# puzzlepaint/camera_calibration

Measured on NVIDIA H100. Metric: LM iterations/sec, higher is better.
Workload: dtype f64

## Files before the change

### camera_calibration_b200/csrc/ba_dense.cu

```cuda

#include <algorithm>
#include <cstdio>
#include <cstdlib>

#include "ba_kernels.h"
#include "ba_tile.cuh"

namespace b200ba {

namespace {

constexpr int BM = 128;
constexpr int LDT = BM + 4;
__host__ __device__ constexpr int gemm_threads(int bn) { return 4 * (bn / 32) * 32; }
constexpr size_t gemm_smem(int bn, int bk, int stages) {
  return static_cast<size_t>(stages) * bk * (LDT + bn + 4) * sizeof(double);
}

__device__ __forceinline__ void cp_async16(void* smem, const void* gmem, int src_bytes) {
  const unsigned s = static_cast<unsigned>(__cvta_generic_to_shared(smem));
  asm volatile("cp.async.cg.shared.global [%0], [%1], 16, %2;\n" ::"r"(s), "l"(gmem), "r"(src_bytes));
}
__device__ __forceinline__ void cp_async8(void* smem, const void* gmem, int src_bytes) {
  const unsigned s = static_cast<unsigned>(__cvta_generic_to_shared(smem));
// ... 598 lines not shown
      bs[row] = v;
    else if (live_row)
      b_below[r] = v;
  }
  if (!chain) return;
  cp_async_wait<0>();
  __syncthreads();
  double s0 = 0.0, s1 = 0.0;
  for (int c = half; c <= row; c += 4) {
    s0 = fma(ts2_smem[c * TS2_LD + row], bs[c], s0);
    if (c + 2 <= row) s1 = fma(ts2_smem[(c + 2) * TS2_LD + row], bs[c + 2], s1);
  }
  part[half][row] = s0 + s1;
  __syncthreads();
  if (half == 0 && live_row) y_next[row] = part[0][row] + part[1][row];
}

__global__ void __launch_bounds__(TS2_THREADS, 1)
    trsv_backward2_kernel(const double* __restrict__ Lpack, const int64_t* __restrict__ panel_off,
                          const int* __restrict__ panel_h, int NB, int r0, int live, const double* __restrict__ x_t,
                          double* __restrict__ y , const double* __restrict__ Linv_prev,
                          double* __restrict__ x_prev ) {
  extern __shared__ __align__(16) double ts2_smem[];
  __shared__ double xs[PT], ysm[PT], part[2][PT];
  const int tid = threadIdx.x;
  const bool chain = blockIdx.x == 0;
  if (chain) stage_tile_async(ts2_smem, Linv_prev);
  if (tid < PT) xs[tid] = (tid < live) ? x_t[tid] : 0.0;
  __syncthreads();
  const int warp = tid >> 5, lane = tid & 31;
  const int cbase = r0 - PT * (static_cast<int>(blockIdx.x) + 1);
#pragma unroll
  for (int batch = 0; batch < 2; ++batch) {
    double l[8][4];
#pragma unroll
    for (int q = 0; q < 8; ++q) {
      const int c = cbase + warp * 16 + batch * 8 + q;
      const int k = c / NB;
      const double* col = Lpack + panel_off[k] + static_cast<int64_t>(c - k * NB) * panel_h[k] + (r0 - k * NB);
#pragma unroll
      for (int u = 0; u < 4; ++u) l[q][u] = (lane + 32 * u < live) ? col[lane + 32 * u] : 0.0;
    }
#pragma unroll
    for (int q = 0; q < 8; ++q) {
      double acc = 0.0;
#pragma unroll
      for (int u = 0; u < 4; ++u) acc = fma(l[q][u], xs[lane + 32 * u], acc);
#pragma unroll
      for (int o = 16; o > 0; o >>= 1) acc += __shfl_xor_sync(0xffffffffu, acc, o);
      if (lane == 0) {
        const int c = cbase + warp * 16 + batch * 8 + q;
        const double v = y[c] - acc;
        if (chain)
          ysm[c - cbase] = v;
        else
          y[c] = v;
      }
    }
  }
  if (!chain) return;
  cp_async_wait<0>();
  __syncthreads();
  const int j = tid & (PT - 1), half = tid >> 7;
  double s0 = 0.0, s1 = 0.0;
  const double* colj = ts2_smem + j * TS2_LD;
  for (int i = j + half; i < PT; i += 4) {
    s0 = fma(colj[i], ysm[i], s0);
    if (i + 2 < PT) s1 = fma(colj[i + 2], ysm[i + 2], s1);
  }
  part[half][j] = s0 + s1;
  __syncthreads();
  if (half == 0) x_prev[j] = part[0][j] + part[1][j];
}

static int panel_version() {
  static int v = -1;
  if (v < 0) v = getenv("B200BA_PANEL") ? atoi(getenv("B200BA_PANEL")) : 2;
  return v;
}
static bool aux_enabled() {
  static const bool v = !(getenv("B200BA_AUX") && atoi(getenv("B200BA_AUX")) == 0);
  return v;
}
static int trsv_version() {
  static int v = -1;
  if (v < 0) v = getenv("B200BA_TRSV") ? atoi(getenv("B200BA_TRSV")) : 2;
  return v;
}

void dense_variants(int* gemm, int* panel, int* trsv, int* aux) {
  *gemm = gemm_variant();
  *panel = panel_version();
  *trsv = trsv_version();
  *aux = aux_enabled() ? 1 : 0;
}

int dense_plan(DenseCtx* d, int n, int nb, int rank, int ranks) {
  d->n = n;
  d->rank = rank;
  d->ranks = ranks;
  d->NB = nb;
  d->nblk = (n + nb - 1) / nb;
  d->ntiles = (n + PT - 1) / PT;
  d->map.nb = nb;
  d->map.ranks = ranks;
  d->map.blocks_per_rank = (d->nblk + ranks - 1) / ranks;
  d->map.ld = (n + 1) / 2 * 2;
  d->chunk = static_cast<int64_t>(d->map.blocks_per_rank) * nb * d->map.ld;
  d->panel_off.assign(d->nblk + 1, 0);
  d->panel_h.assign(std::max(1, d->nblk), 0);
  for (int k = 0; k < d->nblk; ++k) {
    const int hk = n - k * nb;
    d->panel_h[k] = (hk + 1) / 2 * 2;
    d->panel_off[k + 1] = d->panel_off[k] + static_cast<int64_t>(d->panel_h[k]) * nb + static_cast<int64_t>(nb / PT) * PT * PT;
  }
  return 0;
}

int dense_factor(DenseCtx* d) {
  const int n = d->n, NB = d->NB, R = d->ranks, me = d->rank;
  if (n == 0) return 0;
  const int sub_n = NB / PT;
  cudaStream_t sm = d->s_main, sp = d->s_panel;
  auto owner = [&](int k) { return k % R; };
  const bool use_aux = aux_enabled() && R == 1 && d->s_aux != nullptr;
  cudaEventRecord(d->ev_misc, sm);
  cudaStreamWaitEvent(sp, d->ev_misc, 0);

  auto update = [&](int k, int j_first, int j_last, cudaStream_t st, bool owned_only) -> int {
    if (j_first >= d->nblk || j_first > j_last) return 0;
    const int k0 = k * NB, kw = std::min(NB, n - k0);
    const int j0 = j_first * NB;
    const int jn = std::min(n, (std::min(j_last, d->nblk - 1) + 1) * NB) - j0;
    if (jn <= 0) return 0;
    GemmArgs g{};
    g.M = n - j0;
    g.N = jn;
    g.K = kw;
    g.A = d->Lpack + d->panel_off[k] + (j0 - k0);
    g.lda = d->panel_h[k];
    g.B = g.A;
    g.ldb = g.lda;
    g.alpha = -1.0;
    g.beta = 1.0;
    g.a_aligned = g.b_aligned = gemm_operand_aligned(g.A, g.lda);
    if (owned_only) {
      g.C = d->S;
      g.map = d->map;
      g.owned_only = true;
      g.rank = me;
      g.col_base = j0;
    } else {
      g.C = d->S + d->map.col_offset(j0) + j0;
      g.ldc = d->map.ld;
    }
    return launch_dgemm_nt(g, true, false, st, false, true);
  };

  for (int k = 0; k < d->nblk; ++k) {
    const int k0 = k * NB, kw = std::min(NB, n - k0), hk = d->panel_h[k], hlive = n - k0;
    double* P = d->Lpack + d->panel_off[k];
    if (owner(k) == me && panel_version() == 2) {
      const double* Sk = d->S + d->map.col_offset(k0) + k0;
      double* Sk_w = d->S + d->map.col_offset(k0) + k0;
      const int64_t ld = d->map.ld;
      for (int sub = 0; sub < sub_n; ++sub) {
        const int c0 = sub * PT;
        if (c0 >= kw) break;
        const int live = std::min(PT, kw - c0);
        double* tile_out = P + static_cast<int64_t>(c0) * hk + c0;
        double* Li = P + static_cast<int64_t>(hk) * NB + static_cast<int64_t>(sub) * PT * PT;
        if (launch_potrf_trinv_tile(Sk + static_cast<int64_t>(c0) * ld + c0, ld, live, tile_out, hk, Li, d->info, sp)) return 1;
        const int below = hlive - c0 - PT;
        if (below > 0) {
          GemmArgs g{};
          g.M = below;
          g.N = PT;
          g.K = PT;
          g.A = Sk + static_cast<int64_t>(c0) * ld + c0 + PT;
          g.lda = ld;
          g.B = Li;
          g.ldb = PT;
          g.C = tile_out + PT;
          g.ldc = hk;
          g.alpha = 1.0;
          g.beta = 0.0;
          g.a_aligned = gemm_operand_aligned(g.A, g.lda);
          g.b_aligned = gemm_operand_aligned(g.B, g.ldb);
          if (launch_dgemm_nt(g, false, false, sp, false, true)) return 1;
          const int rest = kw - c0 - PT;
          if (rest > 0) {
            GemmArgs u{};
            u.M = below;
            u.N = rest;
            u.K = PT;
            u.A = tile_out + PT;
            u.lda = hk;
            u.B = u.A;
            u.ldb = hk;
            u.C = Sk_w + static_cast<int64_t>(c0 + PT) * ld + (c0 + PT);
            u.ldc = ld;
            u.alpha = -1.0;
            u.beta = 1.0;
            u.a_aligned = u.b_aligned = gemm_operand_aligned(u.A, u.lda);
            if (launch_dgemm_nt(u, true, false, sp, false, true)) return 1;
          }
        }
      }
    } else if (owner(k) == me) {
      cudaMemcpy2DAsync(P, static_cast<size_t>(hk) * sizeof(double), d->S + d->map.col_offset(k0) + k0,
                        static_cast<size_t>(d->map.ld) * sizeof(double), static_cast<size_t>(hlive) * sizeof(double), kw,
                        cudaMemcpyDeviceToDevice, sp);
      for (int sub = 0; sub < sub_n; ++sub) {
        const int c0 = sub * PT;
        if (c0 >= kw) break;
        const int live = std::min(PT, kw - c0);
        double* tile = P + static_cast<int64_t>(c0) * hk + c0;
        double* Li = P + static_cast<int64_t>(hk) * NB + static_cast<int64_t>(sub) * PT * PT;
        if (launch_potrf_tile(tile, hk, live, Li, d->info, sp)) return 1;
        const int below = hlive - c0 - PT;
        if (below > 0) {
          GemmArgs g{};
          g.M = below;
          g.N = PT;
          g.K = PT;
          g.A = tile + PT;
          g.lda = hk;
          g.B = Li;
          g.ldb = PT;
          g.C = tile + PT;
          g.ldc = hk;
          g.alpha = 1.0;
          g.beta = 0.0;
          g.in_place = true;
          g.a_aligned = gemm_operand_aligned(g.A, g.lda);
          g.b_aligned = gemm_operand_aligned(g.B, g.ldb);
          if (launch_dgemm_nt(g, false, false, sp)) return 1;
          const int rest = kw - c0 - PT;
          if (rest > 0) {
            GemmArgs u{};
            u.M = below;
            u.N = rest;
            u.K = PT;
            u.A = tile + PT;
            u.lda = hk;
            u.B = u.A;
            u.ldb = hk;
            u.C = P + static_cast<int64_t>(c0 + PT) * hk + (c0 + PT);
            u.ldc = hk;
            u.alpha = -1.0;
            u.beta = 1.0;
            u.a_aligned = u.b_aligned = gemm_operand_aligned(u.A, u.lda);
            if (launch_dgemm_nt(u, true, false, sp)) return 1;
          }
        }
      }
    }
    if (R > 1) {
      if (d->bcast(P, static_cast<size_t>(hk) * NB + static_cast<size_t>(sub_n) * PT * PT, owner(k), sp, d->user)) return 1;
    }
    cudaEventRecord(d->ev_ready[k & 1], sp);
    cudaStreamWaitEvent(sm, d->ev_ready[k & 1], 0);
    if (k + 3 < d->nblk && update(k, k + 3, d->nblk - 1, sm, R > 1)) return 1;
    cudaEventRecord(d->ev_main[k & 1], sm);
    if (use_aux) {
      if (k >= 1) cudaStreamWaitEvent(sp, d->ev_half2[(k - 1) & 1], 0);
      if (k + 1 < d->nblk && update(k, k + 1, k + 1, sp, false)) return 1;
      if (k + 2 < d->nblk) {
        cudaStreamWaitEvent(d->s_aux, d->ev_ready[k & 1], 0);
        if (k > 0) cudaStreamWaitEvent(d->s_aux, d->ev_main[(k - 1) & 1], 0);
        if (update(k, k + 2, k + 2, d->s_aux, false)) return 1;
      }
      cudaEventRecord(d->ev_half2[k & 1], d->s_aux);
      continue;
    }
    if (k + 1 < d->nblk && owner(k + 1) == me && update(k, k + 1, k + 1, sp, false)) return 1;
    if (k + 2 < d->nblk && owner(k + 2) == me) {
      if (k > 0) cudaStreamWaitEvent(sp, d->ev_main[(k - 1) & 1], 0);
      if (update(k, k + 2, k + 2, sp, false)) return 1;
    }
  }
  if (use_aux && d->nblk >= 1) cudaStreamWaitEvent(sp, d->ev_half2[(d->nblk - 1) & 1], 0);
  cudaEventRecord(d->ev_misc, sp);
  cudaStreamWaitEvent(sm, d->ev_misc, 0);
  return cudaGetLastError() == cudaSuccess ? 0 : 1;
}

int dense_solve(DenseCtx* d, double* b) {
  const int n = d->n, NB = d->NB;
  if (n == 0) return 0;
  cudaStream_t sm = d->s_main;
  const int sub_n = NB / PT;
  auto linv_of = [&](int t) {
    const int k = (t * PT) / NB, sub = (t * PT - k * NB) / PT;
    return d->Lpack + d->panel_off[k] + static_cast<int64_t>(d->panel_h[k]) * NB + static_cast<int64_t>(sub) * PT * PT;
  };
  if (trsv_version() == 2) {
    static bool configured_dev[64] = {};
    int dev = 0;
    cudaGetDevice(&dev);
    if (!configured_dev[dev & 63]) {
      cudaFuncSetAttribute(trsv_forward2_kernel, cudaFuncAttributeMaxDynamicSharedMemorySize, static_cast<int>(kTs2Smem));
      cudaFuncSetAttribute(trsv_backward2_kernel, cudaFuncAttributeMaxDynamicSharedMemorySize, static_cast<int>(kTs2Smem));
      configured_dev[dev & 63] = true;
    }
    const int T = d->ntiles;
    trsv_store_tile_kernel<<<1, PT, 0, sm>>>(linv_of(0), b, std::min(PT, n), d->tmp, false);
    for (int t = 0; t + 1 < T; ++t) {
      const int c0 = t * PT, k = c0 / NB, off = c0 - k * NB;
      const int rows_below = n - c0 - PT;
      const double* Lp = d->Lpack + d->panel_off[k] + static_cast<int64_t>(off) * d->panel_h[k] + off + PT;
      trsv_forward2_kernel<<<(rows_below + PT - 1) / PT, TS2_THREADS, kTs2Smem, sm>>>(Lp, d->panel_h[k], rows_below, d->tmp + c0,
                                                                                      b + c0 + PT, linv_of(t + 1), d->tmp + c0 + PT);
    }
    {
      const int r0 = (T - 1) * PT;
      trsv_store_tile_kernel<<<1, PT, 0, sm>>>(linv_of(T - 1), d->tmp + r0, std::min(PT, n - r0), b + r0, true);
    }
    for (int t = T - 1; t >= 1; --t) {
      const int r0 = t * PT, live = std::min(PT, n - r0);
      trsv_backward2_kernel<<<r0 / PT, TS2_THREADS, kTs2Smem, sm>>>(d->Lpack, d->d_panel_off, d->d_panel_h, NB, r0, live, b + r0,
                                                                    d->tmp, linv_of(t - 1), b + r0 - PT);
    }
    return cudaGetLastError() == cudaSuccess ? 0 : 1;
  }
  for (int t = 0; t < d->ntiles; ++t) {
    const int c0 = t * PT, live = std::min(PT, n - c0), k = c0 / NB;
    const int rows_below = n - c0 - PT;
    const double* Li = linv_of(t);
    if (rows_below > 0) {
      const int grid = (rows_below + TS_ROWS - 1) / TS_ROWS;
      trsv_forward_step_kernel<<<grid, TS_THREADS, 0, sm>>>(d->Lpack + d->panel_off[k], d->panel_h[k], c0 - k * NB, live,
                                                              rows_below, Li, b + c0, d->tmp + c0);
    } else {
      trsv_store_tile_kernel<<<1, PT, 0, sm>>>(Li, b + c0, live, d->tmp + c0, false);
    }
  }
  for (int t = d->ntiles - 1; t >= 0; --t) {
    const int r0 = t * PT, live = std::min(PT, n - r0);
    const double* Li = linv_of(t);
    if (r0 > 0) {
      const int grid = (r0 + TS_THREADS / 32 - 1) / (TS_THREADS / 32);
      trsv_backward_step_kernel<<<grid, TS_THREADS, 0, sm>>>(d->Lpack, d->d_panel_off, d->d_panel_h, NB, r0, live, r0, Li,
                                                               d->tmp + r0, d->tmp, b + r0);
    } else {
      trsv_store_tile_kernel<<<1, PT, 0, sm>>>(Li, d->tmp + r0, live, b + r0, true);
    }
  }
  return cudaGetLastError() == cudaSuccess ? 0 : 1;
}
// ... 58 lines not shown
```

### camera_calibration_b200/csrc/ba_host.cu

```cuda

#include <cublas_v2.h>
#include <cusolverDn.h>
#include <dlfcn.h>

#include <algorithm>
#include <cmath>
#include <cstdarg>
#include <cstdio>
#include <cstring>
#include <limits>
#include <string>
#include <vector>

#include "ba_kernels.h"

using namespace b200ba;

namespace {

std::string g_create_error;

struct NcclUniqueId {
  char internal[128];
};
// ... 59 lines not shown

  std::vector<b200ba_camera> cams_host;
  ProblemDev pb{};
  int n_cameras = 0, n_imagesets = 0, n_points = 0;
  int64_t n_obs = 0;
  int uniform_model = -1;
  int64_t n_control_total = 0, n_param_total = 0, intr_total = 0, tan_total = 0;
  uint32_t *d_obs_imageset = nullptr, *d_obs_camera = nullptr, *d_obs_point = nullptr;
  float2* d_obs_xy = nullptr;

  StateDev st[2]{};
  int cur = 0;
  double2* d_last_projection = nullptr;
  bool have_state = false;
  StateDev snap{};
  double2* d_snap_lp = nullptr;
  bool have_snapshot = false;

  Layout L{};
  bool have_layout = false;
  ObsOut out{};
  ObsOut out_trial{};
  SystemDev sys{};
  double *d_W = nullptr, *d_S = nullptr, *d_Linv = nullptr, *d_v = nullptr, *d_y = nullptr, *d_x = nullptr;
  double trace_H = 0;
  int64_t reduce_count = 0;
  double* d_potrf_work = nullptr;
  int potrf_lwork = 0;
  int chol_mode = -1;
  int chol_nb = 512;
  int *d_info = nullptr, *d_fail = nullptr;
  std::vector<uint32_t> perm;
  uint32_t* d_perm = nullptr;
  double2* d_lp_stage = nullptr;
  uint32_t* d_straggler_list = nullptr;
  int* d_straggler_count = nullptr;
  double *d_partial = nullptr, *d_scal = nullptr;
  double* d_rot = nullptr;
  double* h_scal = nullptr;
  int* h_flags = nullptr;

  std::vector<uint32_t> h_obs_imageset, h_obs_camera, h_obs_point;
  std::vector<float> h_obs_xy;
  int group_blocks_n = 0;
  int n_groups = 0;
  std::vector<int> group_start;
  std::vector<int> group_count;
  int* d_group_of_block = nullptr;
  int* d_group_blocks = nullptr;
  uint8_t* d_flags = nullptr;
  int* d_cols = nullptr;
  int* d_count = nullptr;
  int* h_count = nullptr;
  double* d_Wc = nullptr;
  double* d_P = nullptr;
  size_t wc_stride = 0, p_stride = 0;
  cudaEvent_t ev_syrk[2] = {nullptr, nullptr}, ev_scatter[2] = {nullptr, nullptr}, ev_s_ready = nullptr;
  double* d_u = nullptr;
  bool use_grouped = false;
  double* capture_S = nullptr;
  double* capture_rhs = nullptr;
  std::vector<int32_t> lm_events;
  std::vector<double> grp_sums;
  int force_grouped = -1;
  bool compact_j = true;

  ReportDev rep{};
  double2* d_rep_stage = nullptr;
  bool have_report = false;
  std::vector<int64_t> img_cam_groups;
  int* d_img_group_off = nullptr;
  uint32_t* d_img_group_obs = nullptr;
  bool have_images = false;

  void* comm = nullptr;
  int rank = 0, n_ranks = 1;

  bool own_dense = true;
  DenseCtx dn;
  int dense_planned_ranks = 0, dense_planned_n = -1;
  int dense_nb = 0;
  cudaStream_t panel_stream = nullptr;
  cudaStream_t aux_stream = nullptr;
  int* d_ident_cols = nullptr;
  double* d_gemv_partial = nullptr;

  b200ba_timings timings{};
  struct Pending {
    int phase;
    cudaEvent_t a, b;
    bool own_a = true;
  };
  std::vector<Pending> pending;
  std::vector<cudaEvent_t> event_pool;
};

namespace {

#define CUDA_TRY(h, expr)                                                                      \
  do {                                                                                         \
    cudaError_t _e = (expr);                                                                   \
    if (_e != cudaSuccess) {                                                                   \
      (h)->error = std::string(#expr) + ": " + cudaGetErrorString(_e);                         \
      return 1;                                                                                \
    }                                                                                          \
  } while (0)
#define CUBLAS_TRY(h, expr)                                                                    \
  do {                                                                                         \
    cublasStatus_t _s = (expr);                                                                \
    if (_s != CUBLAS_STATUS_SUCCESS) {                                                         \
      (h)->error = std::string(#expr) + ": cuBLAS status " + std::to_string(static_cast<int>(_s)); \
      return 1;                                                                                \
    }                                                                                          \
  } while (0)
#define CUSOLVER_TRY(h, expr)                                                                  \
  do {                                                                                         \
    cusolverStatus_t _s = (expr);                                                              \
    if (_s != CUSOLVER_STATUS_SUCCESS) {                                                       \
      (h)->error = std::string(#expr) + ": cuSOLVER status " + std::to_string(static_cast<int>(_s)); \
      return 1;                                                                                \
    }                                                                                          \
  } while (0)

template <class T>
int dev_alloc(b200ba_handle* h, T** p, size_t count) {
  if (*p) {
    cudaFree(*p);
    *p = nullptr;
  }
  if (count == 0) count = 1;
  CUDA_TRY(h, cudaMalloc(reinterpret_cast<void**>(p), count * sizeof(T)));
  return 0;
}

int64_t intrinsics_size(const b200ba_camera& c) {
  const int64_t G = static_cast<int64_t>(c.grid_width) * c.grid_height;
  switch (c.model_type) {
    case B200BA_MODEL_CENTRAL_GENERIC: return 3 * G;
    case B200BA_MODEL_NONCENTRAL_GENERIC: return 6 * G;
    default: return 12;
  }
}
int update_parameter_count(const b200ba_camera& c) {
  const int G = c.grid_width * c.grid_height;
  switch (c.model_type) {
    case B200BA_MODEL_CENTRAL_GENERIC: return 2 * G;
    case B200BA_MODEL_NONCENTRAL_GENERIC: return 5 * G;
    default: return 12;
  }
}
int jacobian_size(const b200ba_camera& c) {
  switch (c.model_type) {
    case B200BA_MODEL_CENTRAL_GENERIC: return 32;
    case B200BA_MODEL_NONCENTRAL_GENERIC: return 80;
    default: return 12;
  }
}

void fill_camdev(const b200ba_camera& c, CamDev* d) {
  d->model_type = c.model_type;
  d->width = c.width;
  d->height = c.height;
  d->min_x = c.calibration_min_x;
  d->min_y = c.calibration_min_y;
  d->max_x = c.calibration_max_x;
  d->max_y = c.calibration_max_y;
// ... 71 lines not shown
  cudaFree(d);
  if (rc != 0 || ce != cudaSuccess) {
    h->error = "all-reduce of the group centroids failed";
    return 1;
  }
  return 0;
}

int build_groups(b200ba_handle* h, bool allocate) {
  const Layout& L = h->L;
  const int nb = L.nblocks;
  int gb = (L.bs == 3) ? 96 : 48;
  if (const char* e = getenv("B200BA_GROUP_BLOCKS")) gb = std::max(1, atoi(e));
  h->group_blocks_n = gb;
  std::vector<int> order(nb);
  for (int i = 0; i < nb; ++i) order[i] = i;
  if (L.eliminate_points && nb > 0) {
    const double* sx = h->grp_sums.data();
    const double* sy = sx + nb;
    const double* cnt = sy + nb;
    const double qx = std::max(1.0, h->cams_host[0].width / 64.0), qy = std::max(1.0, h->cams_host[0].height / 64.0);
    std::vector<uint32_t> zkey(nb, 0);
    for (int p = 0; p < nb; ++p) {
      if (cnt[p] <= 0) continue;
      uint32_t ux = static_cast<uint32_t>(std::min(1023.0, std::max(0.0, sx[p] / cnt[p] / qx)));
      uint32_t uy = static_cast<uint32_t>(std::min(1023.0, std::max(0.0, sy[p] / cnt[p] / qy)));
      uint32_t z = 0;
      for (int b = 0; b < 10; ++b) z |= ((ux >> b) & 1u) << (2 * b) | ((uy >> b) & 1u) << (2 * b + 1);
      zkey[p] = z;
    }
    std::stable_sort(order.begin(), order.end(), [&](int a, int b) { return zkey[a] < zkey[b]; });
  }
  h->n_groups = (nb + gb - 1) / gb;
  h->group_start.assign(h->n_groups + 1, 0);
  std::vector<int> gob(std::max(1, nb), 0);
  for (int g = 0; g < h->n_groups; ++g) {
    h->group_start[g] = g * gb;
    for (int i = g * gb; i < std::min(nb, (g + 1) * gb); ++i) gob[order[i]] = g;
  }
  h->group_start[h->n_groups] = nb;
  h->group_count.assign(std::max(1, h->n_groups), 0);
  if (allocate) {
    if (dev_alloc(h, &h->d_group_of_block, std::max(1, nb))) return 1;
    if (dev_alloc(h, &h->d_group_blocks, std::max(1, nb))) return 1;
    if (dev_alloc(h, &h->d_flags, static_cast<size_t>(std::max(1, h->n_groups)) * std::max(1, L.nd))) return 1;
    if (dev_alloc(h, &h->d_cols, static_cast<size_t>(std::max(1, h->n_groups)) * std::max(1, L.nd))) return 1;
    if (dev_alloc(h, &h->d_count, std::max(1, h->n_groups))) return 1;
    if (h->h_count) cudaFreeHost(h->h_count);
    CUDA_TRY(h, cudaMallocHost(reinterpret_cast<void**>(&h->h_count), std::max(1, h->n_groups) * sizeof(int)));
    h->wc_stride = static_cast<size_t>(gb) * L.bs * (std::max(1, L.nd) + 1);
    h->p_stride = static_cast<size_t>(std::max(1, L.nd)) * std::max(1, L.nd);
    if (dev_alloc(h, &h->d_Wc, 2 * h->wc_stride)) return 1;
    if (!h->own_dense && dev_alloc(h, &h->d_P, 2 * h->p_stride)) return 1;
    for (int i = 0; i < 2; ++i) {
      if (!h->ev_syrk[i]) CUDA_TRY(h, cudaEventCreateWithFlags(&h->ev_syrk[i], cudaEventDisableTiming));
      if (!h->ev_scatter[i]) CUDA_TRY(h, cudaEventCreateWithFlags(&h->ev_scatter[i], cudaEventDisableTiming));
    }
    if (!h->ev_s_ready) CUDA_TRY(h, cudaEventCreateWithFlags(&h->ev_s_ready, cudaEventDisableTiming));
    if (dev_alloc(h, &h->d_u, std::max(1, L.nbd))) return 1;
  }
  CUDA_TRY(h, cudaMemcpy(h->d_group_of_block, gob.data(), std::max(1, nb) * sizeof(int), cudaMemcpyHostToDevice));
  if (nb > 0) CUDA_TRY(h, cudaMemcpy(h->d_group_blocks, order.data(), nb * sizeof(int), cudaMemcpyHostToDevice));
  return 0;
}

int nccl_bcast_cb(double* buf, size_t count, int root, cudaStream_t s, void* user) {
  b200ba_handle* h = static_cast<b200ba_handle*>(user);
  const int rc = g_nccl.Broadcast(buf, buf, count, kNcclDouble, root, h->comm, s);
  if (rc != 0) {
    h->error = std::string("ncclBroadcast: ") + (g_nccl.GetErrorString ? g_nccl.GetErrorString(rc) : "error");
    return 1;
  }
  return 0;
}

cudaError_t dense_create(DenseCtx* d, bool own_streams) {
  cudaError_t e = cudaSuccess;
  if (own_streams) {
    int lo = 0, hi = 0;
    cudaDeviceGetStreamPriorityRange(&lo, &hi);
    e = cudaStreamCreateWithFlags(&d->s_main, cudaStreamNonBlocking);
    if (e == cudaSuccess) e = cudaStreamCreateWithPriority(&d->s_panel, cudaStreamNonBlocking, hi);
    if (e == cudaSuccess) e = cudaStreamCreateWithPriority(&d->s_aux, cudaStreamNonBlocking, hi);
  }
  for (cudaEvent_t* ev : {&d->ev_ready[0], &d->ev_ready[1], &d->ev_main[0], &d->ev_main[1], &d->ev_half2[0],
                          &d->ev_half2[1], &d->ev_misc})
    if (e == cudaSuccess && !*ev) e = cudaEventCreateWithFlags(ev, cudaEventDisableTiming);
  return e;
}
void dense_release(DenseCtx* d, bool own_streams) {
  for (cudaEvent_t ev : {d->ev_ready[0], d->ev_ready[1], d->ev_main[0], d->ev_main[1], d->ev_half2[0], d->ev_half2[1],
                         d->ev_misc})
    if (ev) cudaEventDestroy(ev);
  if (own_streams)
    for (cudaStream_t s : {d->s_main, d->s_panel, d->s_aux})
      if (s) cudaStreamDestroy(s);
}

int plan_dense(b200ba_handle* h) {
  if (!h->own_dense || !h->have_layout) return 0;
  const int nd = h->L.nd;
  if (h->dense_planned_n == nd && h->dense_planned_ranks == h->n_ranks) return 0;
  DenseCtx& d = h->dn;
  const int nb = h->dense_nb > 0 ? h->dense_nb : (h->n_ranks == 1 ? 512 : 256);
  dense_plan(&d, nd, nb, h->rank, h->n_ranks);
  if (dev_alloc(h, &h->d_S, static_cast<size_t>(std::max<int64_t>(1, d.chunk * h->n_ranks)))) return 1;
  d.S = h->d_S;
  if (dev_alloc(h, &d.Lpack, static_cast<size_t>(std::max<int64_t>(1, d.panel_off[d.nblk])))) return 1;
  if (dev_alloc(h, &d.tmp, std::max(1, nd))) return 1;
  if (dev_alloc(h, &d.d_panel_off, d.panel_off.size())) return 1;
  if (dev_alloc(h, &d.d_panel_h, d.panel_h.size())) return 1;
  CUDA_TRY(h, cudaMemcpy(d.d_panel_off, d.panel_off.data(), d.panel_off.size() * sizeof(int64_t), cudaMemcpyHostToDevice));
  CUDA_TRY(h, cudaMemcpy(d.d_panel_h, d.panel_h.data(), d.panel_h.size() * sizeof(int), cudaMemcpyHostToDevice));
  {
    std::vector<int> ident(std::max(1, nd));
    for (int i = 0; i < nd; ++i) ident[i] = i;
    if (dev_alloc(h, &h->d_ident_cols, ident.size())) return 1;
    CUDA_TRY(h, cudaMemcpy(h->d_ident_cols, ident.data(), ident.size() * sizeof(int), cudaMemcpyHostToDevice));
  }
  if (dev_alloc(h, &h->d_gemv_partial, static_cast<size_t>(gemv_t_partial_size(h->L.nbd, std::max(1, nd))))) return 1;
  CUDA_TRY(h, cudaMemset(h->d_S, 0, static_cast<size_t>(std::max<int64_t>(1, d.chunk * h->n_ranks)) * sizeof(double)));
  d.info = h->d_info;
  d.s_main = h->stream;
  d.s_panel = h->panel_stream;
  d.s_aux = h->aux_stream;
  CUDA_TRY(h, dense_create(&d, false));
  d.bcast = nccl_bcast_cb;
  d.user = h;
  h->dense_planned_n = nd;
  h->dense_planned_ranks = h->n_ranks;
  return 0;
}

int make_layout(b200ba_handle* h, const b200ba_options* opt) {
  if (opt->regularization_weight != 0) {
    static bool warned = false;
    if (!warned) fprintf(stderr, "[b200ba] regularization_weight is ignored (the term is disabled in the reference, joint_optimization.cc:299-305)\n");
    warned = true;
  }
  Layout L{};
  memset(&L, 0, sizeof(L));
  L.n_points = h->n_points;
  L.n_imagesets = h->n_imagesets;
  L.n_cameras = h->n_cameras;
  L.rig_in_state = h->n_cameras > 1;
  L.localize_only = opt->localize_only ? 1 : 0;
  L.eliminate_points = opt->eliminate_points ? 1 : 0;
  int n_intr = 0, kmax = 0;
  for (int c = 0; c < h->n_cameras; ++c) {
    n_intr += update_parameter_count(h->cams_host[c]);
    kmax = std::max(kmax, jacobian_size(h->cams_host[c]));
  }
  if (L.localize_only) {
    n_intr = 0;
    kmax = 0;
  }
  const int rig_dof = L.rig_in_state ? 6 * h->n_cameras : 0;
  if (L.eliminate_points) {
    L.bs = 3;
    L.nblocks = h->n_points;
    L.g_point = 0;
    L.g_pose = 3 * h->n_points;
    L.g_rig = L.g_pose + 6 * h->n_imagesets;
    L.g_intr = L.g_rig + rig_dof;
  } else {
    L.bs = 6;
    L.nblocks = h->n_imagesets;
    L.g_pose = 0;
    L.g_rig = 6 * h->n_imagesets;
    L.g_point = L.g_rig + rig_dof;
    L.g_intr = L.g_point + 3 * h->n_points;
  }
  L.dsz = L.bs * (L.bs + 1) / 2;
  L.nbd = L.bs * L.nblocks;
  L.dof = 3 * h->n_points + 6 * h->n_imagesets + rig_dof + n_intr;
  L.nd = L.dof - L.nbd;
  L.Kmax = kmax;
  L.jc_point = 0;
  L.jc_pose = 3;
  L.jc_rig = 9;
  L.jc_intr = 9 + (L.rig_in_state ? 6 : 0);
  L.n_jcols = L.jc_intr + kmax;
  const bool same = h->have_layout && memcmp(&L, &h->L, sizeof(Layout)) == 0;
  if (same) return plan_dense(h);
  h->L = L;
  h->have_layout = true;
  h->dense_planned_n = -1;

  const int64_t n = h->n_obs;
  if (dev_alloc(h, &h->out.residual, 2 * n)) return 1;
  if (dev_alloc(h, &h->out.cost, n)) return 1;
  h->out.compact = (h->uniform_model == B200BA_MODEL_CENTRAL_GENERIC && h->compact_j) ? 1 : 0;
  if (h->out.compact) {
    if (h->out.jac) cudaFree(h->out.jac);
    h->out.jac = nullptr;
    if (dev_alloc(h, &h->out.cjac, 14 * static_cast<size_t>(n))) return 1;
  } else {
    if (dev_alloc(h, &h->out.jac, 2 * static_cast<size_t>(L.n_jcols) * n)) return 1;
  }
  if (dev_alloc(h, &h->out.cell, n)) return 1;
  if (dev_alloc(h, &h->out.has_jac, n)) return 1;
  if (dev_alloc(h, &h->out.evals, n)) return 1;
  h->out_trial.evals = nullptr;
  if (dev_alloc(h, &h->out_trial.residual, 2 * n)) return 1;
  if (dev_alloc(h, &h->out_trial.cost, n)) return 1;
  h->out_trial.jac = nullptr;
  h->out_trial.cjac = nullptr;
  h->out_trial.compact = 0;
// ... 915 lines not shown
  }
  cublasSetStream(h->cublas, h->stream);
  if (cusolverDnCreate(&h->cusolver) != CUSOLVER_STATUS_SUCCESS) {
    h->error = "cusolverDnCreate failed";
    return fail(1);
  }
  cusolverDnSetStream(h->cusolver, h->stream);

  h->n_cameras = p->n_cameras;
  h->n_imagesets = p->n_imagesets;
  h->n_points = p->n_points;
  h->n_obs = p->n_obs;
  h->cams_host.assign(p->cameras, p->cameras + p->n_cameras);
  h->uniform_model = h->cams_host[0].model_type;
  int upd = 0;
  for (int c = 0; c < p->n_cameras; ++c) {
    CamDev& d = h->pb.cams[c];
    fill_camdev(h->cams_host[c], &d);
    d.intr_off = h->intr_total;
    d.tan_off = h->tan_total;
    d.upd_off = upd;
    upd += d.upd_count;
    h->intr_total += intrinsics_size(h->cams_host[c]);
    const int64_t G = static_cast<int64_t>(d.gw) * d.gh;
    h->tan_total += 6 * G;
    h->n_control_total += G;
    if (d.gw == 0) h->n_param_total += 12;
    if (h->cams_host[c].model_type != h->uniform_model) h->uniform_model = -1;
  }
  const int64_t n = p->n_obs;
  TRYC(dev_alloc(h, &h->d_obs_imageset, n));
  TRYC(dev_alloc(h, &h->d_obs_camera, n));
  TRYC(dev_alloc(h, &h->d_obs_point, n));
  TRYC(dev_alloc(h, &h->d_obs_xy, n));
  if (n > 0) {
    std::vector<uint32_t> key(n);
    for (int64_t o = 0; o < n; ++o) {
      const uint32_t cam = p->obs_camera[o];
      const CamDev& cd = h->pb.cams[cam];
      uint32_t cell = 0;
      if (cd.gw > 0) {
        const double gx = 1.0 + cd.gmul_x * (static_cast<double>(p->obs_xy[2 * o]) - cd.min_x);
        const double gy = 1.0 + cd.gmul_y * (static_cast<double>(p->obs_xy[2 * o + 1]) - cd.min_y);
        const int x0 = std::min(std::max(static_cast<int>(std::floor(gx)) - 1, 0), cd.gw - 4);
        const int y0 = std::min(std::max(static_cast<int>(std::floor(gy)) - 1, 0), cd.gh - 4);
        cell = static_cast<uint32_t>(x0 + y0 * cd.gw);
      }
      key[o] = (cam << 24) | cell;
    }
    h->perm.resize(n);
    for (int64_t o = 0; o < n; ++o) h->perm[o] = static_cast<uint32_t>(o);
    std::stable_sort(h->perm.begin(), h->perm.end(), [&](uint32_t a, uint32_t b) { return key[a] < key[b]; });
    std::vector<uint32_t> t32(n);
    std::vector<float> txy(2 * n);
    for (int64_t i = 0; i < n; ++i) t32[i] = p->obs_imageset[h->perm[i]];
    TRYC(cuda_ok(cudaMemcpy(h->d_obs_imageset, t32.data(), n * sizeof(uint32_t), cudaMemcpyHostToDevice), "H2D"));
    for (int64_t i = 0; i < n; ++i) t32[i] = p->obs_camera[h->perm[i]];
    TRYC(cuda_ok(cudaMemcpy(h->d_obs_camera, t32.data(), n * sizeof(uint32_t), cudaMemcpyHostToDevice), "H2D"));
    for (int64_t i = 0; i < n; ++i) t32[i] = p->obs_point[h->perm[i]];
    TRYC(cuda_ok(cudaMemcpy(h->d_obs_point, t32.data(), n * sizeof(uint32_t), cudaMemcpyHostToDevice), "H2D"));
    for (int64_t i = 0; i < n; ++i) {
      txy[2 * i] = p->obs_xy[2 * h->perm[i]];
      txy[2 * i + 1] = p->obs_xy[2 * h->perm[i] + 1];
    }
    TRYC(cuda_ok(cudaMemcpy(h->d_obs_xy, txy.data(), n * sizeof(float2), cudaMemcpyHostToDevice), "H2D"));
    TRYC(dev_alloc(h, &h->d_perm, n));
    TRYC(cuda_ok(cudaMemcpy(h->d_perm, h->perm.data(), n * sizeof(uint32_t), cudaMemcpyHostToDevice), "H2D"));
  }
  TRYC(dev_alloc(h, &h->d_lp_stage, n));
  if (n > 0) {
    h->h_obs_imageset.assign(p->obs_imageset, p->obs_imageset + n);
    h->h_obs_camera.assign(p->obs_camera, p->obs_camera + n);
    h->h_obs_point.assign(p->obs_point, p->obs_point + n);
    h->h_obs_xy.assign(p->obs_xy, p->obs_xy + 2 * n);
  }
  if (const char* e = getenv("B200BA_DENSE")) h->own_dense = !(strcmp(e, "lib") == 0 || strcmp(e, "0") == 0);
  if (const char* e = getenv("B200BA_DENSE_NB")) h->dense_nb = std::max(128, atoi(e) / 128 * 128);
  set_gemm_sm_reserve(getenv("B200BA_PANEL_SMS") ? atoi(getenv("B200BA_PANEL_SMS")) : 8);
  {
    int lo = 0, hi = 0;
    cudaDeviceGetStreamPriorityRange(&lo, &hi);
    TRYC(cuda_ok(cudaStreamCreateWithPriority(&h->panel_stream, cudaStreamNonBlocking, hi), "cudaStreamCreate"));
    TRYC(cuda_ok(cudaStreamCreateWithPriority(&h->aux_stream, cudaStreamNonBlocking, hi), "cudaStreamCreate"));
  }
  if (const char* e = getenv("B200BA_GROUPED")) h->force_grouped = atoi(e);
  if (const char* e = getenv("B200BA_COMPACT_J")) h->compact_j = atoi(e) != 0;
  if (const char* e = getenv("B200BA_DIST_CHOL")) h->chol_mode = atoi(e);
  if (const char* e = getenv("B200BA_CHOL_NB")) h->chol_nb = std::max(32, atoi(e));
  h->pb.n_obs = n;
  h->pb.obs_imageset = h->d_obs_imageset;
  h->pb.obs_camera = h->d_obs_camera;
  h->pb.obs_point = h->d_obs_point;
  h->pb.obs_xy = h->d_obs_xy;
  for (int i = 0; i < 2; ++i) {
    TRYC(dev_alloc(h, &h->st[i].points, 3 * static_cast<size_t>(h->n_points)));
    TRYC(dev_alloc(h, &h->st[i].rig_tr_global, 7 * static_cast<size_t>(h->n_imagesets)));
    TRYC(dev_alloc(h, &h->st[i].camera_tr_rig, 7 * static_cast<size_t>(h->n_cameras)));
    TRYC(dev_alloc(h, &h->st[i].intrinsics, h->intr_total));
    TRYC(dev_alloc(h, &h->st[i].image_tr_global, 12 * static_cast<size_t>(h->n_imagesets) * h->n_cameras));
    TRYC(dev_alloc(h, &h->st[i].tangents, h->tan_total));
  }
  TRYC(dev_alloc(h, &h->d_last_projection, n));
  TRYC(cuda_ok(cudaMemset(h->d_last_projection, 0, std::max<int64_t>(1, n) * sizeof(double2)), "memset"));
  TRYC(dev_alloc(h, &h->d_straggler_list, n));
  TRYC(dev_alloc(h, &h->d_straggler_count, 1));
  TRYC(dev_alloc(h, &h->d_info, 2 + kMaxCholPanels));
  TRYC(dev_alloc(h, &h->d_fail, 1));
  TRYC(dev_alloc(h, &h->d_partial, cost_reduce_partial_size()));
  TRYC(dev_alloc(h, &h->d_scal, 16));
  TRYC(cuda_ok(cudaMallocHost(reinterpret_cast<void**>(&h->h_scal), 16 * sizeof(double)), "cudaMallocHost"));
  TRYC(cuda_ok(cudaMallocHost(reinterpret_cast<void**>(&h->h_flags), 4 * sizeof(int)), "cudaMallocHost"));
#undef TRYC
  *out = h;
  return 0;
}

void b200ba_destroy(b200ba_handle* h) {
  if (!h) return;
  cudaSetDevice(h->device);
  if (h->stream) cudaStreamSynchronize(h->stream);
  if (h->comm && g_nccl.CommDestroy) g_nccl.CommDestroy(h->comm);
  resolve_timings(h);
  for (auto e : h->event_pool) cudaEventDestroy(e);
  for (int i = 0; i < 2; ++i) {
    if (h->ev_syrk[i]) cudaEventDestroy(h->ev_syrk[i]);
    if (h->ev_scatter[i]) cudaEventDestroy(h->ev_scatter[i]);
  }
  if (h->ev_s_ready) cudaEventDestroy(h->ev_s_ready);
  free_handle_buffers(h);
  if (h->cublas) cublasDestroy(h->cublas);
  if (h->cusolver) cusolverDnDestroy(h->cusolver);
  if (h->stream) cudaStreamDestroy(h->stream);
  if (h->side_stream) cudaStreamDestroy(h->side_stream);
  if (h->panel_stream) cudaStreamDestroy(h->panel_stream);
  if (h->aux_stream) cudaStreamDestroy(h->aux_stream);
  dense_release(&h->dn, false);
  delete h;
}

int b200ba_set_state(b200ba_handle* h, const b200ba_state* s) {
  if (!h) return 1;
  if (!s || !s->points || !s->rig_tr_global || !s->camera_tr_rig || !s->intrinsics) {
    h->error = "NULL state array";
    return 2;
  }
  CUDA_TRY(h, cudaSetDevice(h->device));
  StateDev& d = h->st[h->cur];
  CUDA_TRY(h, cudaMemcpyAsync(d.points, s->points, 3 * sizeof(double) * h->n_points, cudaMemcpyHostToDevice, h->stream));
  CUDA_TRY(h, cudaMemcpyAsync(d.rig_tr_global, s->rig_tr_global, 7 * sizeof(double) * h->n_imagesets, cudaMemcpyHostToDevice, h->stream));
  CUDA_TRY(h, cudaMemcpyAsync(d.camera_tr_rig, s->camera_tr_rig, 7 * sizeof(double) * h->n_cameras, cudaMemcpyHostToDevice, h->stream));
  for (int c = 0; c < h->n_cameras; ++c)
    CUDA_TRY(h, cudaMemcpyAsync(d.intrinsics + h->pb.cams[c].intr_off, s->intrinsics[c],
                                sizeof(double) * intrinsics_size(h->cams_host[c]), cudaMemcpyHostToDevice, h->stream));
  if (s->last_projection) {
    CUDA_TRY(h, cudaMemcpyAsync(h->d_lp_stage, s->last_projection, 2 * sizeof(double) * h->n_obs, cudaMemcpyHostToDevice, h->stream));
    launch_permute_double2(h->n_obs, h->d_perm, h->d_lp_stage, h->d_last_projection, false, h->stream);
  } else
    CUDA_TRY(h, cudaMemsetAsync(h->d_last_projection, 0, std::max<int64_t>(1, h->n_obs) * sizeof(double2), h->stream));
  CUDA_TRY(h, cudaStreamSynchronize(h->stream));
  h->have_state = true;
  return 0;
}

int b200ba_get_state(b200ba_handle* h, b200ba_state* s) {
  if (!h) return 1;
  if (!s || !h->have_state) {
    h->error = "no state";
    return 2;
  }
  CUDA_TRY(h, cudaSetDevice(h->device));
  const StateDev& d = h->st[h->cur];
  if (s->points) CUDA_TRY(h, cudaMemcpyAsync(s->points, d.points, 3 * sizeof(double) * h->n_points, cudaMemcpyDeviceToHost, h->stream));
  if (s->rig_tr_global) CUDA_TRY(h, cudaMemcpyAsync(s->rig_tr_global, d.rig_tr_global, 7 * sizeof(double) * h->n_imagesets, cudaMemcpyDeviceToHost, h->stream));
  if (s->camera_tr_rig) CUDA_TRY(h, cudaMemcpyAsync(s->camera_tr_rig, d.camera_tr_rig, 7 * sizeof(double) * h->n_cameras, cudaMemcpyDeviceToHost, h->stream));
  if (s->intrinsics)
    for (int c = 0; c < h->n_cameras; ++c)
      CUDA_TRY(h, cudaMemcpyAsync(s->intrinsics[c], d.intrinsics + h->pb.cams[c].intr_off,
                                  sizeof(double) * intrinsics_size(h->cams_host[c]), cudaMemcpyDeviceToHost, h->stream));
  if (s->last_projection) {
    launch_permute_double2(h->n_obs, h->d_perm, h->d_last_projection, h->d_lp_stage, true, h->stream);
    CUDA_TRY(h, cudaMemcpyAsync(s->last_projection, h->d_lp_stage, 2 * sizeof(double) * h->n_obs, cudaMemcpyDeviceToHost, h->stream));
  }
  CUDA_TRY(h, cudaStreamSynchronize(h->stream));
  return 0;
}

static int copy_state_dev(b200ba_handle* h, const StateDev& src, const double2* src_lp, StateDev& dst, double2* dst_lp) {
  CUDA_TRY(h, cudaMemcpyAsync(dst.points, src.points, 3 * sizeof(double) * h->n_points, cudaMemcpyDeviceToDevice, h->stream));
  CUDA_TRY(h, cudaMemcpyAsync(dst.rig_tr_global, src.rig_tr_global, 7 * sizeof(double) * h->n_imagesets, cudaMemcpyDeviceToDevice, h->stream));
  CUDA_TRY(h, cudaMemcpyAsync(dst.camera_tr_rig, src.camera_tr_rig, 7 * sizeof(double) * h->n_cameras, cudaMemcpyDeviceToDevice, h->stream));
  CUDA_TRY(h, cudaMemcpyAsync(dst.intrinsics, src.intrinsics, sizeof(double) * h->intr_total, cudaMemcpyDeviceToDevice, h->stream));
  CUDA_TRY(h, cudaMemcpyAsync(dst_lp, src_lp, sizeof(double2) * std::max<int64_t>(1, h->n_obs), cudaMemcpyDeviceToDevice, h->stream));
  CUDA_TRY(h, cudaStreamSynchronize(h->stream));
  return 0;
}

int b200ba_snapshot_state(b200ba_handle* h) {
  if (!h) return 1;
  if (!h->have_state) {
    h->error = "no state";
    return 2;
  }
  CUDA_TRY(h, cudaSetDevice(h->device));
  if (!h->snap.points) {
    if (dev_alloc(h, &h->snap.points, 3 * static_cast<size_t>(h->n_points))) return 1;
    if (dev_alloc(h, &h->snap.rig_tr_global, 7 * static_cast<size_t>(h->n_imagesets))) return 1;
    if (dev_alloc(h, &h->snap.camera_tr_rig, 7 * static_cast<size_t>(h->n_cameras))) return 1;
    if (dev_alloc(h, &h->snap.intrinsics, h->intr_total)) return 1;
    if (dev_alloc(h, &h->d_snap_lp, h->n_obs)) return 1;
  }
  if (copy_state_dev(h, h->st[h->cur], h->d_last_projection, h->snap, h->d_snap_lp)) return 1;
  h->have_snapshot = true;
  return 0;
}

int b200ba_restore_state(b200ba_handle* h) {
  if (!h) return 1;
  if (!h->have_snapshot) {
// ... 2194 lines not shown
```

### camera_calibration_b200/csrc/ba_kernels.h

```cpp
#pragma once
#include <vector>

#include "ba_common.h"

namespace b200ba {

void launch_prepare_state(const ProblemDev& pb, const Layout& L, const StateDev& st, int64_t n_control_total,
                          cudaStream_t s);
void launch_residual_jacobian(int uniform_model, bool jac, const ProblemDev& pb, const Layout& L,
                              const StateDev& st, double2* last_projection, const ObsOut& out, double huber,
                              uint32_t* straggler_list, int* straggler_count, cudaStream_t s,
                              cudaEvent_t main_done = nullptr);
void launch_straggler_pass(int uniform_model, bool jac, const ProblemDev& pb, const Layout& L, const StateDev& st,
                           double2* last_projection, const ObsOut& out, double huber, uint32_t* straggler_list,
                           int* straggler_count, cudaStream_t s);
void launch_accumulate_list(const ProblemDev& pb, const Layout& L, const StateDev& st, const ObsOut& out,
                            const SystemDev& sys, double huber, const uint32_t* list, const int* count, cudaStream_t s);
void launch_expand_jacobian(const ProblemDev& pb, const Layout& L, const StateDev& st, const ObsOut& out, double* jac,
                            cudaStream_t s);
void set_main_eval_budget(int budget);
void launch_accumulate_scatter(const ProblemDev& pb, const Layout& L, const StateDev& st, const ObsOut& out,
                               const SystemDev& sys, double huber, cudaStream_t s);
void launch_accumulate_cells(const ProblemDev& pb, const Layout& L, const StateDev& st, const ObsOut& out,
                             const SystemDev& sys, double huber, cudaStream_t s);
// ... 67 lines not shown
                           cudaStream_t s);
struct RefineParams {
  int w, h;
  int half;
  int n_samples, n_match;
  int type;
  int num_star_segments, squares_x, squares_y, num_tags;
  int4 tags[B200BA_PATTERN_MAX_TAGS];
};
void launch_refine_features(const RefineParams& p, int64_t n, const b200ba_feature_prediction* pred,
                            const uint8_t* images, const float2* samples, float2* xy, float* cost, int* status,
                            cudaStream_t s);
void launch_generic_block_inverse(int bs, int nb, int nd, const double* D, const double* B, const double* b1,
                                  double* DinvB, double* Dinvb, cudaStream_t s);
void launch_symmetrize(int n, double* M, cudaStream_t s);
void launch_dirfit_tangents(int G, const double* grid, double* tan, cudaStream_t s);
void launch_dirfit(bool jac, int gw, int64_t n, const double* gp, const double* dirs, const double* grid,
                   const double* tan, double* H, double* b, int dof, double* cost, double* cost_sum, cudaStream_t s);
void launch_dirfit_update(int G, const double* grid, const double* x, double* out, cudaStream_t s);
void launch_permute_double2(int64_t n, const uint32_t* perm, const double2* src, double2* dst, bool scatter,
                            cudaStream_t s);


void launch_mask_fixed(const Layout& L, const SystemDev& sys, const FixedRanges& fr, double unit, cudaStream_t s);
void launch_nice_orientation(const ProblemDev& pb, const StateDev& st, int n_cameras, double* rot, cudaStream_t s);

struct DenseMap {
  int nb;
  int ranks;
  int blocks_per_rank;
  int64_t ld;
  __host__ __device__ __forceinline__ int slot(int block) const { return (block % ranks) * blocks_per_rank + block / ranks; }
  __host__ __device__ __forceinline__ int64_t col_offset(int c) const {
    const int b = c / nb;
    return (static_cast<int64_t>(slot(b)) * nb + (c - b * nb)) * ld;
  }
};

struct GemmArgs {
  int M, N, K;
  const double* A;
  int64_t lda;
  const double* B;
  int64_t ldb;
  double* C;
  int64_t ldc;
  double alpha, beta;
  bool a_aligned, b_aligned;
  const int* cols;
  DenseMap map;
  int64_t n_tiles_lower;
  bool owned_only;
  int rank, col_base;
  bool in_place;
};
inline bool gemm_operand_aligned(const double* p, int64_t ld) {
  return (reinterpret_cast<uintptr_t>(p) % 16 == 0) && (ld % 2 == 0);
}
int launch_dgemm_nt(const GemmArgs& g, bool lower, bool scatter, cudaStream_t s, bool leave_sms = false,
                    bool one_tile_per_cta = false);
void set_gemm_sm_reserve(int n);
int launch_potrf_tile(double* A, int64_t lda, int n, double* Linv, int* info, cudaStream_t s);

int gemv_t_partial_size(int rows, int cols);
void launch_gemv_t(int rows, int cols, int64_t ld, const double* B, const double* u, double alpha, double* y, double* partial,
                   cudaStream_t s);
void launch_gemv_n(int rows, int cols, int64_t ld, const double* B, const double* x, double* t, cudaStream_t s);
void launch_add_diagonal_map(int n, double* S, const DenseMap& map, double lambda, cudaStream_t s);

struct DenseCtx {
  int n = 0, NB = 256, nblk = 0, ntiles = 0;
  int rank = 0, ranks = 1;
  DenseMap map{};
  int64_t chunk = 0;
  std::vector<int64_t> panel_off;
  std::vector<int> panel_h;
  double* S = nullptr;
  double* Lpack = nullptr;
  double* tmp = nullptr;
  int64_t* d_panel_off = nullptr;
  int* d_panel_h = nullptr;
  int* info = nullptr;
  cudaStream_t s_main = nullptr, s_panel = nullptr, s_aux = nullptr;
  cudaEvent_t ev_ready[2] = {nullptr, nullptr}, ev_main[2] = {nullptr, nullptr}, ev_half2[2] = {nullptr, nullptr}, ev_misc = nullptr;
  int (*bcast)(double* buf, size_t count, int root, cudaStream_t s, void* user) = nullptr;
  void* user = nullptr;
};
int dense_plan(DenseCtx* d, int n, int nb, int rank, int ranks);
int dense_factor(DenseCtx* d);
int dense_solve(DenseCtx* d, double* b);
void dense_variants(int* gemm, int* panel, int* trsv, int* aux);

}
```

Baseline: 23.35.

## Add lookahead stream to overlap panel factorization critical path with trailing updates

Adds a fourth high-priority stream and events so that, inside the dense blocked Cholesky panel factorization, only the first PT-row slice of the triangular solve and update runs on the panel stream. The remaining rows are handled on a lookahead stream. The next-panel trailing update is likewise split, so the next panel's first tile can start as soon as its leading columns are updated. This shortens the serial critical path of small kernels. In exchange it launches more, smaller GEMMs and adds cross-stream event dependencies, which could cost launch overhead or introduce ordering mistakes.

```diff
diff --git a/camera_calibration_b200/csrc/ba_dense.cu b/camera_calibration_b200/csrc/ba_dense.cu
--- a/camera_calibration_b200/csrc/ba_dense.cu
+++ b/camera_calibration_b200/csrc/ba_dense.cu
@@ -704,6 +704,10 @@
   static const bool v = !(getenv("B200BA_AUX") && atoi(getenv("B200BA_AUX")) == 0);
   return v;
 }
+static bool lookahead_enabled() {
+  static const bool v = !(getenv("B200BA_LOOKAHEAD") && atoi(getenv("B200BA_LOOKAHEAD")) == 0);
+  return v;
+}
 static int trsv_version() {
   static int v = -1;
   if (v < 0) v = getenv("B200BA_TRSV") ? atoi(getenv("B200BA_TRSV")) : 2;
@@ -743,9 +747,10 @@
   const int n = d->n, NB = d->NB, R = d->ranks, me = d->rank;
   if (n == 0) return 0;
   const int sub_n = NB / PT;
-  cudaStream_t sm = d->s_main, sp = d->s_panel;
+  cudaStream_t sm = d->s_main, sp = d->s_panel, sl = d->s_look;
   auto owner = [&](int k) { return k % R; };
   const bool use_aux = aux_enabled() && R == 1 && d->s_aux != nullptr;
+  const bool lookahead = lookahead_enabled() && panel_version() == 2 && sl != nullptr;
   cudaEventRecord(d->ev_misc, sm);
   cudaStreamWaitEvent(sp, d->ev_misc, 0);
 
@@ -778,6 +783,25 @@
     }
     return launch_dgemm_nt(g, true, false, st, false, true);
   };
+  auto update_part = [&](int k, int r0, int m, int c0, int nc, bool lower, cudaStream_t st) -> int {
+    if (m <= 0 || nc <= 0) return 0;
+    const int k0 = k * NB;
+    GemmArgs g{};
+    g.M = m;
+    g.N = nc;
+    g.K = std::min(NB, n - k0);
+    g.A = d->Lpack + d->panel_off[k] + (r0 - k0);
+    g.lda = d->panel_h[k];
+    g.B = d->Lpack + d->panel_off[k] + (c0 - k0);
+    g.ldb = g.lda;
+    g.alpha = -1.0;
+    g.beta = 1.0;
+    g.a_aligned = gemm_operand_aligned(g.A, g.lda);
+    g.b_aligned = gemm_operand_aligned(g.B, g.ldb);
+    g.C = d->S + d->map.col_offset(c0) + r0;
+    g.ldc = d->map.ld;
+    return launch_dgemm_nt(g, lower, false, st, false, true);
+  };
 
   for (int k = 0; k < d->nblk; ++k) {
     const int k0 = k * NB, kw = std::min(NB, n - k0), hk = d->panel_h[k], hlive = n - k0;
@@ -794,40 +818,71 @@
         double* Li = P + static_cast<int64_t>(hk) * NB + static_cast<int64_t>(sub) * PT * PT;
         if (launch_potrf_trinv_tile(Sk + static_cast<int64_t>(c0) * ld + c0, ld, live, tile_out, hk, Li, d->info, sp)) return 1;
         const int below = hlive - c0 - PT;
-        if (below > 0) {
+        if (below <= 0) continue;
+        const int rest = kw - c0 - PT;
+        auto solve = [&](int r0, int m, cudaStream_t st) -> int {
+          if (m <= 0) return 0;
           GemmArgs g{};
-          g.M = below;
+          g.M = m;
           g.N = PT;
           g.K = PT;
-          g.A = Sk + static_cast<int64_t>(c0) * ld + c0 + PT;
+          g.A = Sk + static_cast<int64_t>(c0) * ld + c0 + PT + r0;
           g.lda = ld;
           g.B = Li;
           g.ldb = PT;
-          g.C = tile_out + PT;
+          g.C = tile_out + PT + r0;
           g.ldc = hk;
           g.alpha = 1.0;
           g.beta = 0.0;
           g.a_aligned = gemm_operand_aligned(g.A, g.lda);
           g.b_aligned = gemm_operand_aligned(g.B, g.ldb);
-          if (launch_dgemm_nt(g, false, false, sp, false, true)) return 1;
-          const int rest = kw - c0 - PT;
+          return launch_dgemm_nt(g, false, false, st, false, true);
+        };
+        auto upd = [&](int r0, int m, int c_lo, int nc, bool lower, cudaStream_t st) -> int {
+          if (m <= 0 || nc <= 0) return 0;
+          GemmArgs u{};
+          u.M = m;
+          u.N = nc;
+          u.K = PT;
+          u.A = tile_out + PT + r0;
+          u.lda = hk;
+          u.B = tile_out + PT + c_lo;
+          u.ldb = hk;
+          u.C = Sk_w + static_cast<int64_t>(c0 + PT + c_lo) * ld + (c0 + PT + r0);
+          u.ldc = ld;
+          u.alpha = -1.0;
+          u.beta = 1.0;
+          u.a_aligned = gemm_operand_aligned(u.A, u.lda);
+          u.b_aligned = gemm_operand_aligned(u.B, u.ldb);
+          return launch_dgemm_nt(u, lower, false, st, false, true);
+        };
+        if (!lookahead) {
+          if (solve(0, below, sp) || upd(0, below, 0, rest, true, sp)) return 1;
+          continue;
+        }
+        const int m1 = std::min(PT, below), below2 = below - m1;
+        const int n1 = std::min(PT, rest);
+        cudaEventRecord(d->ev_la_tile, sp);
+        cudaStreamWaitEvent(sp, d->ev_la_cols, 0);
+        if (solve(0, m1, sp)) return 1;
+        cudaStreamWaitEvent(sp, d->ev_la_rest, 0);
+        if (upd(0, m1, 0, n1, true, sp)) return 1;
+        cudaEventRecord(d->ev_la_chain, sp);
+        if (below2 > 0) {
+          cudaStreamWaitEvent(sl, d->ev_la_tile, 0);
+          if (solve(m1, below2, sl)) return 1;
           if (rest > 0) {
-            GemmArgs u{};
-            u.M = below;
-            u.N = rest;
-            u.K = PT;
-            u.A = tile_out + PT;
-            u.lda = hk;
-            u.B = u.A;
-            u.ldb = hk;
-            u.C = Sk_w + static_cast<int64_t>(c0 + PT) * ld + (c0 + PT);
-            u.ldc = ld;
-            u.alpha = -1.0;
-            u.beta = 1.0;
-            u.a_aligned = u.b_aligned = gemm_operand_aligned(u.A, u.lda);
-            if (launch_dgemm_nt(u, true, false, sp, false, true)) return 1;
+            cudaStreamWaitEvent(sl, d->ev_la_chain, 0);
+            if (upd(m1, below2, 0, n1, false, sl)) return 1;
+            cudaEventRecord(d->ev_la_cols, sl);
+            if (upd(m1, below2, n1, rest - n1, true, sl)) return 1;
+            cudaEventRecord(d->ev_la_rest, sl);
           }
         }
+      }
+      if (lookahead) {
+        cudaEventRecord(d->ev_la_rest, sl);
+        cudaStreamWaitEvent(sp, d->ev_la_rest, 0);
       }
     } else if (owner(k) == me) {
       cudaMemcpy2DAsync(P, static_cast<size_t>(hk) * sizeof(double), d->S + d->map.col_offset(k0) + k0,
@@ -887,7 +942,18 @@
     cudaEventRecord(d->ev_main[k & 1], sm);
     if (use_aux) {
       if (k >= 1) cudaStreamWaitEvent(sp, d->ev_half2[(k - 1) & 1], 0);
-      if (k + 1 < d->nblk && update(k, k + 1, k + 1, sp, false)) return 1;
+      if (k + 1 < d->nblk && lookahead) {
+        const int j0 = (k + 1) * NB, jn = std::min(NB, n - j0), m1 = std::min(PT, n - j0), n1 = std::min(PT, jn);
+        if (update_part(k, j0, m1, j0, n1, true, sp)) return 1;
+        cudaStreamWaitEvent(sl, d->ev_ready[k & 1], 0);
+        if (k >= 1) cudaStreamWaitEvent(sl, d->ev_half2[(k - 1) & 1], 0);
+        if (update_part(k, j0 + m1, n - j0 - m1, j0, n1, false, sl)) return 1;
+        cudaEventRecord(d->ev_la_cols, sl);
+        if (update_part(k, j0 + m1, n - j0 - m1, j0 + n1, jn - n1, true, sl)) return 1;
+        cudaEventRecord(d->ev_la_rest, sl);
+      } else if (k + 1 < d->nblk && update(k, k + 1, k + 1, sp, false)) {
+        return 1;
+      }
       if (k + 2 < d->nblk) {
         cudaStreamWaitEvent(d->s_aux, d->ev_ready[k & 1], 0);
         if (k > 0) cudaStreamWaitEvent(d->s_aux, d->ev_main[(k - 1) & 1], 0);
diff --git a/camera_calibration_b200/csrc/ba_host.cu b/camera_calibration_b200/csrc/ba_host.cu
--- a/camera_calibration_b200/csrc/ba_host.cu
+++ b/camera_calibration_b200/csrc/ba_host.cu
@@ -165,6 +165,7 @@
   int dense_nb = 0;
   cudaStream_t panel_stream = nullptr;
   cudaStream_t aux_stream = nullptr;
+  cudaStream_t look_stream = nullptr;
   int* d_ident_cols = nullptr;
   double* d_gemv_partial = nullptr;
 
@@ -402,18 +403,19 @@
     e = cudaStreamCreateWithFlags(&d->s_main, cudaStreamNonBlocking);
     if (e == cudaSuccess) e = cudaStreamCreateWithPriority(&d->s_panel, cudaStreamNonBlocking, hi);
     if (e == cudaSuccess) e = cudaStreamCreateWithPriority(&d->s_aux, cudaStreamNonBlocking, hi);
+    if (e == cudaSuccess) e = cudaStreamCreateWithPriority(&d->s_look, cudaStreamNonBlocking, hi);
   }
   for (cudaEvent_t* ev : {&d->ev_ready[0], &d->ev_ready[1], &d->ev_main[0], &d->ev_main[1], &d->ev_half2[0],
-                          &d->ev_half2[1], &d->ev_misc})
+                          &d->ev_half2[1], &d->ev_misc, &d->ev_la_tile, &d->ev_la_chain, &d->ev_la_cols, &d->ev_la_rest})
     if (e == cudaSuccess && !*ev) e = cudaEventCreateWithFlags(ev, cudaEventDisableTiming);
   return e;
 }
 void dense_release(DenseCtx* d, bool own_streams) {
   for (cudaEvent_t ev : {d->ev_ready[0], d->ev_ready[1], d->ev_main[0], d->ev_main[1], d->ev_half2[0], d->ev_half2[1],
-                         d->ev_misc})
+                         d->ev_misc, d->ev_la_tile, d->ev_la_chain, d->ev_la_cols, d->ev_la_rest})
     if (ev) cudaEventDestroy(ev);
   if (own_streams)
-    for (cudaStream_t s : {d->s_main, d->s_panel, d->s_aux})
+    for (cudaStream_t s : {d->s_main, d->s_panel, d->s_aux, d->s_look})
       if (s) cudaStreamDestroy(s);
 }
 
@@ -444,6 +446,7 @@
   d.s_main = h->stream;
   d.s_panel = h->panel_stream;
   d.s_aux = h->aux_stream;
+  d.s_look = h->look_stream;
   CUDA_TRY(h, dense_create(&d, false));
   d.bcast = nccl_bcast_cb;
   d.user = h;
@@ -1525,6 +1528,7 @@
     cudaDeviceGetStreamPriorityRange(&lo, &hi);
     TRYC(cuda_ok(cudaStreamCreateWithPriority(&h->panel_stream, cudaStreamNonBlocking, hi), "cudaStreamCreate"));
     TRYC(cuda_ok(cudaStreamCreateWithPriority(&h->aux_stream, cudaStreamNonBlocking, hi), "cudaStreamCreate"));
+    TRYC(cuda_ok(cudaStreamCreateWithPriority(&h->look_stream, cudaStreamNonBlocking, hi), "cudaStreamCreate"));
   }
   if (const char* e = getenv("B200BA_GROUPED")) h->force_grouped = atoi(e);
   if (const char* e = getenv("B200BA_COMPACT_J")) h->compact_j = atoi(e) != 0;
@@ -1577,6 +1581,7 @@
   if (h->side_stream) cudaStreamDestroy(h->side_stream);
   if (h->panel_stream) cudaStreamDestroy(h->panel_stream);
   if (h->aux_stream) cudaStreamDestroy(h->aux_stream);
+  if (h->look_stream) cudaStreamDestroy(h->look_stream);
   dense_release(&h->dn, false);
   delete h;
 }
diff --git a/camera_calibration_b200/csrc/ba_kernels.h b/camera_calibration_b200/csrc/ba_kernels.h
--- a/camera_calibration_b200/csrc/ba_kernels.h
+++ b/camera_calibration_b200/csrc/ba_kernels.h
@@ -173,7 +173,9 @@
   int* d_panel_h = nullptr;
   int* info = nullptr;
   cudaStream_t s_main = nullptr, s_panel = nullptr, s_aux = nullptr;
+  cudaStream_t s_look = nullptr;
   cudaEvent_t ev_ready[2] = {nullptr, nullptr}, ev_main[2] = {nullptr, nullptr}, ev_half2[2] = {nullptr, nullptr}, ev_misc = nullptr;
+  cudaEvent_t ev_la_tile = nullptr, ev_la_chain = nullptr, ev_la_cols = nullptr, ev_la_rest = nullptr;
   int (*bcast)(double* buf, size_t count, int root, cudaStream_t s, void* user) = nullptr;
   void* user = nullptr;
 };
```

New measurement: 23.52 (median of 6 runs). About the same (+0.7%).
